# fluidex/plonkit

Hardware: AMD Instinct MI355X
Metric: G1 MSM throughput at 2^20 terms per GPU (KZG commitment of the PLONK prover) (higher is better)
Workload: dtype u256 (BN254 Fr/Fq Montgomery; 9x29-bit limbs in registers, v_mad_u64_u32); 1 GPU; Pippenger G1 MSM (KZG commitment), 2^20 uniform scalars per GPU, tau=42 monomial SRS sharded by rank (BASELINE configs[1]); terms_per_gpu=1048576, parallelism=srs-shard x1 + all_gather of partial sums, exchange=none (one GPU), pipeline_depth=3, settle_steps=0, comm_ranks=1

## Files before the change

plonkit_amd/csrc/ec29_dev.h:

```cpp
#pragma once
#include "field29_dev.h"
#include "ec_dev.h"

namespace plk {

struct AffW { FqW9 x, y; };
struct alignas(16) XyzzW { FqW9 x, y, zz, zzz; };

#define WM(a, b) mulw<FqW>((a), (b))
#define WS(a) sqrw<FqW>((a))
#define WMA(a, b, c, d) mul2addw<FqW>((a), (b), (c), (d))
#define LM(a, b) mulw_os<FqW>((a), (b))
#define LS(a) sqrw_os<FqW>((a))
#define LMA(a, b, c, d) mul2addw_os<FqW>((a), (b), (c), (d))

PLK_HD bool is_inf(const XyzzW &p) { return w_all_zero(p.zz); }
PLK_HD bool is_inf(const AffW &p) { return w_all_zero(p.x) && w_all_zero(p.y); }
PLK_HD XyzzW xyzzw_identity() { XyzzW r; r.x = w_zero<FqW>(); r.y = w_zero<FqW>(); r.zz = w_zero<FqW>(); r.zzz = w_zero<FqW>(); return r; }

PLK_HD XyzzW xyzzw_double_affine(const FqW9 &x, const FqW9 &y) {
    FqW9 u = addn(y, y), v = WS(u), w = WM(u, v), s = WM(x, v);
    FqW9 xx = WS(x), m = normw(addw(addw(xx, xx), xx));
    XyzzW r;
    r.x = sub4(WS(m), addn(s, s));
// ... 71 lines not shown
        }
        mulw2_add<FqW>(q.x, acc.zz, ax, yq, acc.zzz, ay, p, r);
    }
    if (maybe_zero_mod_p(p)) {
        AffW t; t.x = q.x; t.y = normw(yq);
        xyzzw_add_mixed_special(acc, t, false, p, r);
        fresh = is_inf(acc);
        return;
    }
    FqW9 pp, rr, ppp, qq;
    sqrw2<FqW>(p, r, pp, rr);
    mulw2<FqW>(p, pp, acc.x, pp, ppp, qq);
    FqW9 x3;
    {
#pragma unroll
        for (int i = 0; i < 9; i++) x3.l[i] = rr.l[i] + FqW::PAD4[i] - ppp.l[i] - 2 * qq.l[i];
        x3 = normw(x3);
    }
    FqW9 zz3, zzz3;
    mulw2<FqW>(acc.zz, pp, acc.zzz, ppp, zz3, zzz3);
    FqW9 t, nppp;
#pragma unroll
    for (int i = 0; i < 9; i++) { t.l[i] = qq.l[i] + FqW::PAD6N[i] - x3.l[i]; nppp.l[i] = FqW::PAD2N[i] - ppp.l[i]; }
    acc.y = WMA(r, t, acc.y, nppp);
    acc.x = x3;
    acc.zz = zz3;
    acc.zzz = zzz3;
}

PLK_HD void xyzzw_add(XyzzW &a, const XyzzW &b) {
    if (is_inf(b)) return;
    if (is_inf(a)) { a = b; return; }
    FqW9 u1 = LM(a.x, b.zz), u2 = LM(b.x, a.zz), s1 = LM(a.y, b.zzz), s2 = LM(b.y, a.zzz);
    FqW9 p = sub2(u2, u1), r = sub2(s2, s1);
    if (is_zero_mod_p(p)) {
        if (is_zero_mod_p(r)) a = xyzzw_double(a);
        else a = xyzzw_identity();
        return;
    }
    FqW9 pp = LS(p), ppp = LM(p, pp), qq = LM(u1, pp);
    FqW9 x3;
    {
        FqW9 rr = LS(r);
#pragma unroll
        for (int i = 0; i < 9; i++) x3.l[i] = rr.l[i] + FqW::PAD4[i] - ppp.l[i] - 2 * qq.l[i];
        x3 = normw(x3);
    }
    a.y = LMA(r, sub6(qq, x3), s1, neg2(ppp));
    a.x = x3;
    a.zz = LM(LM(a.zz, b.zz), pp);
    a.zzz = LM(LM(a.zzz, b.zzz), ppp);
}

__device__ __forceinline__ AffW load_affw(const G1Affine *p) {
    AffW r; r.x = unpack<FqW>(load_fp(&p->x)); r.y = unpack<FqW>(load_fp(&p->y)); return r;
}
__device__ __forceinline__ FqW9 load_w(const uint32_t *p) {
    FqW9 r;
    const u32x4 *q = reinterpret_cast<const u32x4 *>(p);
    u32x4 a = q[0], b = q[1];
    r.l[0] = a.x; r.l[1] = a.y; r.l[2] = a.z; r.l[3] = a.w; r.l[4] = b.x; r.l[5] = b.y; r.l[6] = b.z; r.l[7] = b.w; r.l[8] = p[8];
    return r;
}
__device__ __forceinline__ void store_w(uint32_t *p, const FqW9 &v) {
    u32x4 *q = reinterpret_cast<u32x4 *>(p);
    q[0] = u32x4{v.l[0], v.l[1], v.l[2], v.l[3]};
    q[1] = u32x4{v.l[4], v.l[5], v.l[6], v.l[7]};
    p[8] = v.l[8];
}
__device__ __forceinline__ XyzzW load_xyzzw(const XyzzW *p) {
    const uint32_t *w = reinterpret_cast<const uint32_t *>(p);
    XyzzW r;
    FqW9 *c[4] = {&r.x, &r.y, &r.zz, &r.zzz};
    u32x4 tail = *reinterpret_cast<const u32x4 *>(w + 32);
    const uint32_t t[4] = {tail.x, tail.y, tail.z, tail.w};
#pragma unroll
    for (int k = 0; k < 4; k++) {
        const u32x4 *q = reinterpret_cast<const u32x4 *>(w + 8 * k);
        u32x4 a = q[0], b = q[1];
        c[k]->l[0] = a.x; c[k]->l[1] = a.y; c[k]->l[2] = a.z; c[k]->l[3] = a.w;
        c[k]->l[4] = b.x; c[k]->l[5] = b.y; c[k]->l[6] = b.z; c[k]->l[7] = b.w; c[k]->l[8] = t[k];
    }
    return r;
}
__device__ __forceinline__ void store_xyzzw(XyzzW *p, const XyzzW &v) {
    uint32_t *w = reinterpret_cast<uint32_t *>(p);
    const FqW9 *c[4] = {&v.x, &v.y, &v.zz, &v.zzz};
#pragma unroll
    for (int k = 0; k < 4; k++) {
        u32x4 *q = reinterpret_cast<u32x4 *>(w + 8 * k);
        q[0] = u32x4{c[k]->l[0], c[k]->l[1], c[k]->l[2], c[k]->l[3]};
        q[1] = u32x4{c[k]->l[4], c[k]->l[5], c[k]->l[6], c[k]->l[7]};
    }
    *reinterpret_cast<u32x4 *>(w + 32) = u32x4{v.x.l[8], v.y.l[8], v.zz.l[8], v.zzz.l[8]};
}

__device__ __forceinline__ G1Xyzz xyzzw_export(const XyzzW &p) {
    G1Xyzz r;
    if (is_inf(p)) return xyzz_identity();
    r.x = pack<FqParams>(s_from_w(p.x)); r.y = pack<FqParams>(s_from_w(p.y));
    r.zz = pack<FqParams>(s_from_w(p.zz)); r.zzz = pack<FqParams>(s_from_w(p.zzz));
    return r;
}

}
```

plonkit_amd/csrc/field29_dev.h:

```cpp
#pragma once
#include "field_dev.h"
#include <utility>

namespace plk {

template <int... J, class F> __device__ __forceinline__ void static_for_impl(std::integer_sequence<int, J...>, F &&f) { (f(std::integral_constant<int, J>{}), ...); }
template <int N, class F> __device__ __forceinline__ void static_for(F &&f) { static_for_impl(std::make_integer_sequence<int, N>{}, static_cast<F &&>(f)); }

constexpr uint32_t M29 = (1u << 29) - 1;
constexpr uint32_t MULW_A_LIMB_MAX = 3280000000u;

struct FrW {
    static constexpr uint32_t P29[9] = {0x10000001u, 0x1f0fac9fu, 0x0e5c2450u, 0x07d090f3u, 0x1585d283u, 0x02db40c0u, 0x00a6e141u, 0x0e5c2634u, 0x0030644eu};
    static constexpr uint32_t INV29 = 0x0fffffffu;
    static constexpr uint32_t PINV0 = 0x10000001u;
    static constexpr uint32_t ONE_W[9] = {0x0fffff57u, 0x1ea70ab4u, 0x052c068bu, 0x17504f49u, 0x0aa8075bu, 0x1d4240ceu, 0x11d54c07u, 0x052ac7a8u, 0x000dc836u};
    static constexpr uint32_t W_FROM_S[9] = {0x0fffead7u, 0x1d5444f4u, 0x04438aa5u, 0x03b4d096u, 0x134c84dau, 0x0e92d304u, 0x14cb95b3u, 0x041b9d3du, 0x00058003u};
    static constexpr uint32_t S_FROM_W[9] = {0x0ffffffbu, 0x04b1a0e2u, 0x18334a6bu, 0x18ed2b3eu, 0x1462e36fu, 0x11b7bc3cu, 0x1cbd99bau, 0x183340fbu, 0x000e0a77u};
    static constexpr uint32_t PAD2[9] = {0x80000002u, 0x9e1f593bu, 0x9cb8489du, 0x8fa121e2u, 0x8b0ba502u, 0x85b6817du, 0x814dc27eu, 0x9cb84c64u, 0x0060c898u};
    static constexpr uint32_t PAD4[9] = {0x80000004u, 0x9c3eb27au, 0x9970913fu, 0x9f4243c9u, 0x96174a08u, 0x8b6d02feu, 0x829b8500u, 0x997098ccu, 0x00c19135u};
    static constexpr uint32_t PAD6[9] = {0x80000006u, 0x9a5e0bb9u, 0x9628d9e1u, 0x8ee365b0u, 0x8122ef0fu, 0x91238480u, 0x83e94782u, 0x9628e534u, 0x012259d2u};
    static constexpr uint32_t PAD8[9] = {0x80000008u, 0x987d64f8u, 0x92e12283u, 0x9e848797u, 0x8c2e9415u, 0x96da0601u, 0x85370a04u, 0x92e1319cu, 0x0183226fu};
};

// ... 416 lines not shown
    const uint32_t q = a.l[8] / (WP::P29[8] + 1u);
    W9<WP> r;
    int64_t c = 0;
#pragma unroll
    for (int i = 0; i < 8; i++) {
        const int64_t s = (int64_t)a.l[i] - (int64_t)q * (int64_t)WP::P29[i] + c;
        r.l[i] = (uint32_t)s & M29;
        c = s >> 29;
    }
    r.l[8] = (uint32_t)((int64_t)a.l[8] - (int64_t)q * (int64_t)WP::P29[8] + c);
    return csub_p(r);
}

template <class WP>
PLK_HD bool is_zero_mod_p(const W9<WP> &a) {
    uint32_t k = (a.l[0] * WP::PINV0) & M29;
    if (k >= 16) return false;
    return w_all_zero(reduce_full(a));
}

template <class WP>
PLK_HD bool maybe_zero_mod_p(const W9<WP> &a) { return ((a.l[0] * WP::PINV0) & M29) < 16; }

template <class WP>
PLK_HD W9<WP> mulsum3w(const W9<WP> &a0, const W9<WP> &b0, const W9<WP> &a1, const W9<WP> &b1, const W9<WP> &a2, const W9<WP> &b2) {
    uint32_t m[9];
    W9<WP> r;
    uint64_t acc = 0;
#pragma unroll
    for (int k = 0; k < 9; k++) {
#pragma unroll
        for (int i = 0; i <= k; i++) {
            acc += (uint64_t)a0.l[k - i] * b0.l[i]; PLK_CHAIN(acc); acc += (uint64_t)a1.l[k - i] * b1.l[i]; PLK_CHAIN(acc);
            acc += (uint64_t)a2.l[k - i] * b2.l[i]; PLK_CHAIN(acc);
        }
        PLK_MONT_LOW(k)
    }
#pragma unroll
    for (int k = 9; k < 17; k++) {
#pragma unroll
        for (int i = k - 8; i <= 8; i++) {
            acc += (uint64_t)a0.l[k - i] * b0.l[i]; PLK_CHAIN(acc); acc += (uint64_t)a1.l[k - i] * b1.l[i]; PLK_CHAIN(acc);
            acc += (uint64_t)a2.l[k - i] * b2.l[i]; PLK_CHAIN(acc);
        }
        PLK_MONT_HIGH(k)
    }
    r.l[8] = (uint32_t)acc;
    return r;
}

template <class WP> PLK_HD W9<WP> w_from_s(const W9<WP> &raw) { return mulw(raw, w_from_s_const<WP>()); }
template <class WP> PLK_HD W9<WP> s_from_w(const W9<WP> &a) { return csub_p(mulw(a, s_from_w_const<WP>())); }

using FrW9 = W9<FrW>;
using FqW9 = W9<FqW>;

}
```

plonkit_amd/csrc/msm.hip:

```cpp
#include "msm_shape.h"
#include "msm.h"
#include "ec29_quad_dev.h"
#include "comm.h"
#include "hostmath.h"
#include <cstring>
#include <cstdlib>

namespace plk {

int32_t msm_small_launch(plk_ctx::MsmSlot &S, hipStream_t stream, const G1Affine *bases, uint32_t copy_stride, const ScalarSet &set,
                         uint32_t batch, uint32_t n, bool ev_on, void *host_out);
constexpr uint32_t SM_PLANES_HOST = 17;
constexpr uint64_t MSM_SMALL_MAX = 1ull << 15;
constexpr uint64_t MSM_OWNED_MAX = 1ull << 16;

__global__ void __launch_bounds__(MSM_THREADS) msm_digits(ScalarSet set, MsmParams p, int32_t *digits) {
    const uint32_t i = blockIdx.x * MSM_THREADS + threadIdx.x, m = blockIdx.y;
    if (i >= p.n) return;
    Fr k = to_canonical(load_fp(set.v[m] + i));
    uint32_t carry = 0;
    const uint32_t half = 1u << (p.c - 1);
    int32_t *out = digits + (size_t)m * p.windows * p.n + i;
    for (uint32_t w = 0; w < p.windows; w++) {
        uint32_t v = extract_bits(k.l, w * p.c, p.c) + carry;
// ... 68 lines not shown
        lcnt[b] = 0;
    }
    __syncthreads();
#pragma unroll
    for (uint32_t k = 0; k < PER; k++) {
        const int32_t d = dreg[k];
        if (d) {
            const uint32_t i = first + tid + k * PART_THREADS;
            uint32_t mg = (uint32_t)(d < 0 ? -d : d) - 1, bin = mg >> p.fine_bits;
            staged[lstart[bin] + atomicAdd(&lcnt[bin], 1u)] = ((copy_tag | i) << 8) | (d < 0 ? 0x80u : 0u) | (mg & ((1u << p.fine_bits) - 1));
        }
    }
    __syncthreads();
    copy_out_runs<PART_THREADS>(lstart, gbase, staged, entries, p.nbins);
}

__global__ void __launch_bounds__(1024) msm_scan_bins(uint32_t *hist, uint32_t *bin_start, uint32_t *task_start, uint32_t total_bins) {
    __shared__ uint32_t sums[1024], tsums[1024];
    const uint32_t tid = threadIdx.x;
    const uint32_t per = (total_bins + 1023) / 1024;
    uint32_t lo = tid * per, hi = lo + per < total_bins ? lo + per : total_bins, s = 0, ts = 0;
    if (lo > total_bins) lo = total_bins;
    for (uint32_t i = lo; i < hi; i++) { s += hist[i]; ts += (hist[i] + TASK_MAX - 1) / TASK_MAX; }
    sums[tid] = s; tsums[tid] = ts;
    __syncthreads();
    for (uint32_t off = 1; off < 1024; off <<= 1) {
        uint32_t v = tid >= off ? sums[tid - off] : 0, tv = tid >= off ? tsums[tid - off] : 0;
        __syncthreads();
        sums[tid] += v; tsums[tid] += tv;
        __syncthreads();
    }
    uint32_t run = tid ? sums[tid - 1] : 0, trun = tid ? tsums[tid - 1] : 0;
    for (uint32_t i = lo; i < hi; i++) {
        uint32_t c = hist[i];
        bin_start[i] = run; run += c;
        task_start[i] = trun; trun += (c + TASK_MAX - 1) / TASK_MAX;
        hist[i] = 0;
    }
    if (tid == 1023) { bin_start[total_bins] = sums[1023]; task_start[total_bins] = tsums[1023]; }
}

constexpr int RC_THREADS = 1024, RC_SCALARS = 1024;
static_assert(RC_WINDOWS == 254 / 17 + 1, "the fused path is the c = 17 shape");

__device__ __forceinline__ bool wave_same_scalar(const Fr &k, bool live, uint64_t live_mask) {
    const int leader = __ffsll((unsigned long long)live_mask) - 1;
    uint32_t diff = 0;
#pragma unroll
    for (int i = 0; i < 8; i++) diff |= k.l[i] ^ (uint32_t)__shfl((int)k.l[i], leader);
    return __ballot(live && diff != 0) == 0;
}

constexpr int RC_COUNT_PER = 4;
__global__ void __launch_bounds__(RC_THREADS) msm_recode_count(ScalarSet set, MsmParams p, uint32_t *hist) {
    __shared__ uint32_t lcnt[1024];
    const uint32_t tid = threadIdx.x, m = blockIdx.y;
    lcnt[tid] = 0;
    __syncthreads();
    Fr k[RC_COUNT_PER];
    bool live[RC_COUNT_PER];
#pragma unroll
    for (int r = 0; r < RC_COUNT_PER; r++) {
        const uint32_t i = (blockIdx.x * RC_COUNT_PER + r) * RC_THREADS + tid;
        live[r] = i < p.n;
        if (live[r]) k[r] = load_fp(set.v[m] + i);
    }
#pragma unroll
    for (int r = 0; r < RC_COUNT_PER; r++) {
        const uint64_t lv = __ballot(live[r]);
        if (!lv) continue;
        const bool same = wave_same_scalar(k[r], live[r], lv);
        if (!live[r]) continue;
        int32_t d[RC_WINDOWS];
        recode17(to_canonical(k[r]), d);
        if (same) {
            if ((tid & 63) == (uint32_t)(__ffsll((unsigned long long)lv) - 1)) {
#pragma unroll
                for (uint32_t w = 0; w < RC_WINDOWS; w++)
                    if (d[w]) { const uint32_t mg = (uint32_t)(d[w] < 0 ? -d[w] : d[w]) - 1; atomicAdd(&lcnt[mg >> p.fine_bits], (uint32_t)__popcll(lv)); }
            }
            continue;
        }
#pragma unroll
        for (uint32_t w = 0; w < RC_WINDOWS; w++)
            if (d[w]) { const uint32_t mg = (uint32_t)(d[w] < 0 ? -d[w] : d[w]) - 1; atomicAdd(&lcnt[mg >> p.fine_bits], 1u); }
    }
    __syncthreads();
    if (tid < p.nbins && lcnt[tid]) atomicAdd(&hist[m * p.nbins + tid], lcnt[tid]);
}

__global__ void __launch_bounds__(RC_THREADS) msm_recode_scatter(ScalarSet set, MsmParams p, uint32_t *cursor, const uint32_t *bin_start, uint32_t *entries) {
    extern __shared__ __attribute__((aligned(16))) char smem[];
    uint32_t *lcnt = reinterpret_cast<uint32_t *>(smem);
    uint32_t *lstart = lcnt + p.nbins;
    uint32_t *gbase = lstart + p.nbins + 1;
    uint32_t *staged = gbase + p.nbins;
    const uint32_t tid = threadIdx.x, m = blockIdx.y;
    const uint32_t i = blockIdx.x * RC_SCALARS + tid;
    cursor += m * p.nbins; bin_start += m * p.nbins;
    int32_t d[RC_WINDOWS];
    const bool live = i < p.n;
    const uint64_t lv = __ballot(live);
    bool same = false;
    uint32_t lane_rank = 0, wave_live = 0;
    if (live) {
        const Fr k = load_fp(set.v[m] + i);
        same = wave_same_scalar(k, true, lv);
        recode17(to_canonical(k), d);
        lane_rank = (uint32_t)__popcll(lv & ((1ull << (tid & 63)) - 1)); wave_live = (uint32_t)__popcll(lv);
    } else {
#pragma unroll
        for (uint32_t w = 0; w < RC_WINDOWS; w++) d[w] = 0;
    }
    for (uint32_t b = tid; b < p.nbins; b += RC_THREADS) lcnt[b] = 0;
    __syncthreads();
    uint32_t at[RC_WINDOWS];
#pragma unroll
    for (uint32_t w = 0; w < RC_WINDOWS; w++) {
        at[w] = 0;
        if (d[w]) {
            const uint32_t mg = (uint32_t)(d[w] < 0 ? -d[w] : d[w]) - 1;
            if (!same) at[w] = atomicAdd(&lcnt[mg >> p.fine_bits], 1u);
            else {
                uint32_t base = 0;
                if (lane_rank == 0) base = atomicAdd(&lcnt[mg >> p.fine_bits], wave_live);
                at[w] = (uint32_t)__shfl((int)base, __ffsll((unsigned long long)lv) - 1) + lane_rank;
            }
        }
    }
    __syncthreads();
    {
        const uint32_t cnt = tid < p.nbins ? lcnt[tid] : 0;
        uint32_t v = cnt;
        for (int off = 1; off < 64; off <<= 1) { uint32_t t = __shfl_up(v, off); if ((int)(tid & 63) >= off) v += t; }
        uint32_t *wtot = gbase;
        if ((tid & 63) == 63) wtot[tid >> 6] = v;
        __syncthreads();
        uint32_t before = 0;
        for (uint32_t w = 0; w < (tid >> 6); w++) before += wtot[w];
        __syncthreads();
        const uint32_t reserved = cnt ? bin_start[tid] + atomicAdd(&cursor[tid], cnt) : 0;
        if (tid < p.nbins) lstart[tid] = before + v - cnt;
        if (tid == RC_THREADS - 1) lstart[p.nbins] = before + v;
        __syncthreads();
        if (tid < p.nbins) gbase[tid] = reserved;
    }
    const uint32_t fmask = (1u << p.fine_bits) - 1;
#pragma unroll
    for (uint32_t w = 0; w < RC_WINDOWS; w++) {
        if (!d[w]) continue;
        const uint32_t mg = (uint32_t)(d[w] < 0 ? -d[w] : d[w]) - 1, bin = mg >> p.fine_bits;
        staged[lstart[bin] + at[w]] = ((((uint32_t)w << p.nbits) | i) << 8) | (d[w] < 0 ? 0x80u : 0u) | (mg & fmask);
    }
    __syncthreads();
    copy_out_runs<RC_THREADS>(lstart, gbase, staged, entries, p.nbins);
}

__device__ __forceinline__ XyzzW shfl_xor_w(const XyzzW &v, int mask) {
    XyzzW r;
#pragma unroll
    for (int i = 0; i < 9; i++) {
// ... 129 lines not shown
        PLK_HIP(hipMemsetAsync(found.p, 0, sizeof(uint32_t), stream));
        hipLaunchKernelGGL(table_find_inf_kernel, dim3(fblocks), dim3(256), 0, stream, (const G1Affine *)table, total, found.as<uint32_t>());
        hipError_t e = hipMemcpyAsync(&found_host, found.p, sizeof(uint32_t), hipMemcpyDeviceToHost, stream);
        if (e == hipSuccess) e = hipStreamSynchronize(stream);
        found.release();
        PLK_HIP(e);
    }
    PLK_HIP(hipGetLastError());
    ctx->srs_w_valid = true;
    ctx->srs_w_copies = copies;
    ctx->srs_w_no_inf = found_host == 0;
    return PLK_OK;
}

static uint32_t slots_per_task(uint32_t fb) { return (1u << fb) + 2 * MSM_THREADS; }
static uint32_t meta_per_task(uint32_t fb) { return (1u << fb) + 2; }

constexpr uint32_t HOT_SPAN = 8;
__device__ __forceinline__ uint32_t bucket_span(const uint32_t *meta, uint32_t b, uint32_t mu) {
    const uint32_t s0 = meta[b], e0 = meta[b + 1];
    return e0 > s0 ? (e0 - 1) / mu - s0 / mu : 0;
}
__device__ __forceinline__ void latency_chain_priority() { __builtin_amdgcn_s_setprio(3); }

template <uint32_t FB, uint32_t RL_LOG>
__global__ void __launch_bounds__(MSM_THREADS) msm_fold_hot(XyzzW *partials, const uint32_t *task_meta, const uint32_t *task_start, uint32_t total_bins) {
    constexpr uint32_t FINE = Shape<FB>::FINE, SLOT_PRIMARY = Shape<FB>::SLOT_PRIMARY, SLOT_HEAD = Shape<FB>::SLOT_HEAD,
                       SLOTS_PER_TASK = Shape<FB>::SLOTS_PER_TASK, META_PER_TASK = Shape<FB>::META_PER_TASK, RL = 1u << RL_LOG, RB = FINE / RL;
    latency_chain_priority();
    const uint32_t gt = blockIdx.x * MSM_THREADS + threadIdx.x;
    const uint32_t task = gt / RL, sub = gt % RL;
    const bool live = task < task_start[total_bins];
    const uint32_t *meta = task_meta + (size_t)(live ? task : 0) * META_PER_TASK;
    const uint32_t nc_raw = live ? meta[FINE + 1] : 0, nc = nc_raw & ~TASK_OWNED_BIT;
    if (!__any(nc != 0 && !(nc_raw & TASK_OWNED_BIT))) return;
    const uint32_t mu = (nc_raw & TASK_OWNED_BIT) ? 0x7fffffffu : (nc ? (nc + MSM_THREADS - 1) / MSM_THREADS : 1);
    uint32_t hot_mask = 0;
    if (nc) for (uint32_t k = 0; k < RB; k++) if (bucket_span(meta, RB * sub + k, mu) > HOT_SPAN) hot_mask |= 1u << k;
    if (!__any(hot_mask != 0)) return;
    XyzzW *P = partials + (size_t)(live ? task : 0) * SLOTS_PER_TASK;
    for (uint32_t owner = 0; owner < RL; owner++) {
        const uint32_t m = __shfl(hot_mask, owner, RL);
        for (uint32_t k = 0; k < RB; k++) {
            if (!((m >> k) & 1)) continue;
            const uint32_t b = RB * owner + k, tf = meta[b] / mu, tl = (meta[b + 1] - 1) / mu;
            XyzzW acc = xyzzw_identity();
            for (uint32_t t = tf + 1 + sub; t <= tl; t += RL) { XyzzW o = load_xyzzw(P + SLOT_HEAD + t); xyzzw_add_nl(acc, o); }
            for (uint32_t x = 1; x < RL; x <<= 1) { XyzzW o = shfl_xor_w(acc, x); xyzzw_add_nl(acc, o); }
            if (sub == 0) store_xyzzw(P + SLOT_PRIMARY + b, acc);
        }
    }
}

template <uint32_t FB, uint32_t RL_LOG>
__global__ void __launch_bounds__(MSM_THREADS, 2) msm_task_reduce(const XyzzW *partials, const uint32_t *task_meta,
                                                                   const uint32_t *task_start, XyzzW *task_out, uint32_t total_bins) {
    constexpr uint32_t FINE = Shape<FB>::FINE, SLOT_PRIMARY = Shape<FB>::SLOT_PRIMARY, SLOT_HEAD = Shape<FB>::SLOT_HEAD, SLOT_TAIL = Shape<FB>::SLOT_TAIL,
                       SLOTS_PER_TASK = Shape<FB>::SLOTS_PER_TASK, META_PER_TASK = Shape<FB>::META_PER_TASK, RL = 1u << RL_LOG, RB = FINE / RL, RB_LOG = FB - RL_LOG;
    static_assert(FB >= RL_LOG + 1, "at least two buckets per lane");
    latency_chain_priority();
    const uint32_t gt = blockIdx.x * MSM_THREADS + threadIdx.x;
    const uint32_t task = gt / RL, sub = gt % RL;
    const bool live = task < task_start[total_bins];
    if (!__any(live)) return;
    const uint32_t *meta = task_meta + (size_t)(live ? task : 0) * META_PER_TASK;
    const uint32_t nc_raw = live ? meta[FINE + 1] : 0, nc = nc_raw & ~TASK_OWNED_BIT;
    const uint32_t mu = (nc_raw & TASK_OWNED_BIT) ? 0x7fffffffu : (nc ? (nc + MSM_THREADS - 1) / MSM_THREADS : 1);
    const XyzzW *P = partials + (size_t)(live ? task : 0) * SLOTS_PER_TASK;
    XyzzW X = xyzzw_identity(), Y = xyzzw_identity();
    uint32_t k = nc ? RB : 0;
    uint32_t piece = 0, piece_end = 0;
    bool pending_sum = false;
    constexpr uint32_t USTEPS = RL_LOG + RB_LOG + 1 + RL_LOG;
    uint32_t ustep = 0;
    for (;;) {
        const bool done = (piece >= piece_end) && !pending_sum && k == 0;
        const bool lockstep = __all(done);
        if (lockstep && ustep == USTEPS) break;
        XyzzW O = xyzzw_identity();
        bool to_y = false;
        if (!lockstep) {
            if (piece < piece_end) { O = load_xyzzw(P + piece); piece++; }
            else if (pending_sum) { to_y = true; pending_sum = false; }
            else if (k > 0) {
                k--;
                const uint32_t b = RB * sub + k, s0 = meta[b], e0 = meta[b + 1];
                if (e0 > s0) {
                    const uint32_t tf = s0 / mu, tl = (e0 - 1) / mu;
                    pending_sum = true;
                    if (tf == tl) O = load_xyzzw(P + SLOT_PRIMARY + b);
                    else {
                        O = load_xyzzw(P + SLOT_TAIL + tf);
                        if (tl - tf > HOT_SPAN) { piece = SLOT_PRIMARY + b; piece_end = piece + 1; }
                        else { piece = SLOT_HEAD + tf + 1; piece_end = SLOT_HEAD + tl + 1; }
                    }
                } else to_y = true;
            }
        } else {
            if (ustep < RL_LOG) {
                const uint32_t off = 1u << ustep;
                O = shfl_down_w(X, off);
                if (sub + off >= RL) O = xyzzw_identity();
            } else {
                if (ustep == RL_LOG) {
                    if (live && sub == 0) store_xyzzw(task_out + 2 * (size_t)task + 1, X);
                    if (sub == 0) X = xyzzw_identity();
                }
                if (ustep < RL_LOG + RB_LOG) O = X;
                else if (ustep == RL_LOG + RB_LOG) O = Y;
                else O = shfl_xor_w(X, 1 << (ustep - RL_LOG - RB_LOG - 1));
            }
            ustep++;
        }
        if (to_y) O = Y;
        XyzzW Tacc = X;
        xyzzw_add(Tacc, O);
        if (to_y) Y = Tacc; else X = Tacc;
    }
    if (live && sub == 0) store_xyzzw(task_out + 2 * (size_t)task, X);
}

template <uint32_t FB>
__global__ void __launch_bounds__(MSM_THREADS) msm_task_reduce_quad(const XyzzW *partials, const uint32_t *task_meta, const uint32_t *task_start, XyzzW *task_out, uint32_t total_bins) {
    constexpr uint32_t FINE = Shape<FB>::FINE, SLOT_PRIMARY = Shape<FB>::SLOT_PRIMARY, SLOT_HEAD = Shape<FB>::SLOT_HEAD, SLOT_TAIL = Shape<FB>::SLOT_TAIL,
                       SLOTS_PER_TASK = Shape<FB>::SLOTS_PER_TASK, META_PER_TASK = Shape<FB>::META_PER_TASK, RL_LOG = 4, RL = 1u << RL_LOG, RB = FINE / RL, RB_LOG = FB - RL_LOG;
    latency_chain_priority();
    const uint32_t task = blockIdx.x * (MSM_THREADS / 64) + (threadIdx.x >> 6), sub = (threadIdx.x & 63u) >> 2, coord = threadIdx.x & 3u;
    const bool live = task < task_start[total_bins];
    if (!live) return;
    const uint32_t *meta = task_meta + (size_t)(live ? task : 0) * META_PER_TASK;
    const uint32_t nc_raw = live ? meta[FINE + 1] : 0, nc = nc_raw & ~TASK_OWNED_BIT;
    const uint32_t mu = (nc_raw & TASK_OWNED_BIT) ? 0x7fffffffu : (nc ? (nc + MSM_THREADS - 1) / MSM_THREADS : 1);
    const XyzzW *P = partials + (size_t)(live ? task : 0) * SLOTS_PER_TASK;
    FqW9 X = w_zero<FqW>(), Y = w_zero<FqW>();
    uint32_t k = nc ? RB : 0;
    uint32_t piece = 0, piece_end = 0;
    bool pending_sum = false;
    constexpr uint32_t USTEPS = RL_LOG + RB_LOG + 1 + RL_LOG;
    uint32_t ustep = 0;
    for (;;) {
        const bool done = (piece >= piece_end) && !pending_sum && k == 0;
        const bool lockstep = __all(done);
        if (lockstep && ustep == USTEPS) break;
        FqW9 O = w_zero<FqW>();
        bool to_y = false;
        if (!lockstep) {
            if (piece < piece_end) { O = load_coord(P + piece, coord); piece++; }
            else if (pending_sum) { to_y = true; pending_sum = false; }
            else if (k > 0) {
                k--;
                const uint32_t b = RB * sub + k, s0 = meta[b], e0 = meta[b + 1];
                if (e0 > s0) {
                    const uint32_t tf = s0 / mu, tl = (e0 - 1) / mu;
                    pending_sum = true;
                    if (tf == tl) O = load_coord(P + SLOT_PRIMARY + b, coord);
                    else {
                        O = load_coord(P + SLOT_TAIL + tf, coord);
                        if (tl - tf > HOT_SPAN) { piece = SLOT_PRIMARY + b; piece_end = piece + 1; }
                        else { piece = SLOT_HEAD + tf + 1; piece_end = SLOT_HEAD + tl + 1; }
                    }
                } else to_y = true;
            }
        } else {
            if (ustep < RL_LOG) {
                const uint32_t off = 1u << ustep;
#pragma unroll
                for (int i = 0; i < 9; i++) O.l[i] = __shfl_down(X.l[i], 4 * off);
                if (sub + off >= RL) O = w_zero<FqW>();
            } else {
// ... 122 lines not shown
    if (S.pinned) (void)hipHostFree(S.pinned);
    S.pinned = nullptr; S.pinned_cap = 0;
    PLK_HIP(hipHostMalloc(&S.pinned, bytes, hipHostMallocDefault));
    S.pinned_cap = bytes;
    return PLK_OK;
}

struct BigArgs { const G1Affine *bases; uint64_t srs_n; uint32_t copies, c_bits, nbits; ScalarSet set; uint32_t batch; uint64_t n; bool no_inf = false; };
static int32_t msm_big_launch(plk_ctx *ctx, plk_ctx::MsmSlot &S, hipStream_t stream, const BigArgs &A) {
    const G1Affine *bases = A.bases;
    const uint32_t batch = A.batch, copies = A.copies;
    const uint64_t n = A.n;
    MsmParams p;
    p.n = (uint32_t)n;
    p.c = A.c_bits;
    p.windows = 254 / p.c + 1;
    p.groups = p.windows / copies;
    p.nbits = A.nbits;
    p.copy_stride = copies > 1 ? (uint32_t)(p.groups * A.srs_n) : 0;
    p.fine_bits = FINE_BITS;
    p.coarse_bits = p.c - 1 - p.fine_bits;
    p.nbins = 1u << p.coarse_bits;
    p.batch = batch;
    const ScalarSet &set = A.set;
    const uint32_t total_sets = batch * p.groups, total_bins = total_sets * p.nbins, total_windows = batch * p.windows;
    const uint32_t max_tasks = total_bins + (uint32_t)(((uint64_t)total_windows * n) / TASK_MAX) + 1;
    PLK_TRY(S.a.reserve((size_t)(3 * total_bins + 4) * sizeof(uint32_t)));
    PLK_TRY(S.b.reserve((size_t)total_windows * n * sizeof(uint32_t)));
    const uint32_t META_PER_TASK = meta_per_task(p.fine_bits), SLOTS_PER_TASK = slots_per_task(p.fine_bits);
    PLK_TRY(S.c.reserve((size_t)max_tasks * 2 * sizeof(XyzzW) + (size_t)max_tasks * META_PER_TASK * 4));
    PLK_TRY(S.e.reserve((size_t)max_tasks * SLOTS_PER_TASK * sizeof(XyzzW)));
    PLK_TRY(S.d.reserve((size_t)13 * total_sets * sizeof(G1Xyzz)));
    uint32_t *hist = S.a.as<uint32_t>(), *bin_start = hist + total_bins, *task_start = bin_start + total_bins + 1;
    uint32_t *entries = S.b.as<uint32_t>();
    XyzzW *task_out = S.c.as<XyzzW>();
    uint32_t *task_meta = reinterpret_cast<uint32_t *>(task_out + 2 * (size_t)max_tasks);
    XyzzW *partials = S.e.as<XyzzW>();
    G1Xyzz *window_out = S.d.as<G1Xyzz>();

    PLK_HIP(hipMemsetAsync(hist, 0, total_bins * sizeof(uint32_t), stream));
    static std::atomic<bool> attr_set{false};
    if (!attr_set) {
        PLK_HIP(hipFuncSetAttribute(reinterpret_cast<const void *>(msm_partition<true>), hipFuncAttributeMaxDynamicSharedMemorySize, 96 * 1024));
        PLK_HIP(hipFuncSetAttribute(reinterpret_cast<const void *>(msm_recode_scatter), hipFuncAttributeMaxDynamicSharedMemorySize, 96 * 1024));
        PLK_TRY(msm_accumulate_prepare());
        attr_set = true;
    }
    static const bool fused_ok = [] { const char *e = getenv("PLK_MSM_FUSED_RECODE"); return !(e && e[0] == '0'); }();
    const uint32_t shape_prephase = (fused_ok && p.groups == 1 && p.c == 17 && p.windows == RC_WINDOWS && p.nbins <= 1024) ? 1u : 2u;
    if (shape_prephase == 1) {
        const uint32_t cblocks = (uint32_t)((n + (uint64_t)RC_THREADS * RC_COUNT_PER - 1) / ((uint64_t)RC_THREADS * RC_COUNT_PER));
        const uint32_t sblocks = (uint32_t)((n + RC_SCALARS - 1) / RC_SCALARS);
        const size_t lds = (size_t)(3 * p.nbins + 1 + RC_SCALARS * RC_WINDOWS) * sizeof(uint32_t);
        hipLaunchKernelGGL(msm_recode_count, dim3(cblocks, batch), dim3(RC_THREADS), 0, stream, set, p, hist);
        hipLaunchKernelGGL(msm_scan_bins, dim3(1), dim3(1024), 0, stream, hist, bin_start, task_start, total_bins);
        hipLaunchKernelGGL(msm_recode_scatter, dim3(sblocks, batch), dim3(RC_THREADS), lds, stream, set, p, hist, (const uint32_t *)bin_start, entries);
    } else {
        PLK_TRY(S.f.reserve((size_t)total_windows * n * sizeof(int32_t)));
        int32_t *digits = S.f.as<int32_t>();
        hipLaunchKernelGGL(msm_digits, dim3((uint32_t)((n + MSM_THREADS - 1) / MSM_THREADS), batch), dim3(MSM_THREADS), 0, stream, set, p, digits);
        const uint32_t pblocks = (uint32_t)((n + DIGIT_CHUNK - 1) / DIGIT_CHUNK);
        const size_t plds_count = (size_t)p.nbins * sizeof(uint32_t);
        const size_t plds_scatter = (size_t)(3 * p.nbins + 1 + DIGIT_CHUNK) * sizeof(uint32_t);
        hipLaunchKernelGGL(msm_partition<false>, dim3(pblocks, total_windows), dim3(PART_THREADS), plds_count, stream, (const int32_t *)digits, p, hist, (const uint32_t *)nullptr, (uint32_t *)nullptr);
        hipLaunchKernelGGL(msm_scan_bins, dim3(1), dim3(1024), 0, stream, hist, bin_start, task_start, total_bins);
        hipLaunchKernelGGL(msm_partition<true>, dim3(pblocks, total_windows), dim3(PART_THREADS), plds_scatter, stream, (const int32_t *)digits, p, hist, (const uint32_t *)bin_start, entries);
    }
    if (ctx->ev_on) PLK_HIP(hipEventRecord(S.ev[0], stream));
    const uint32_t shape_variant = n <= MSM_OWNED_MAX ? 2u : 0u;
    S.acc_no_inf = shape_variant == 0 && A.no_inf;
    msm_accumulate_launch((int)shape_variant, S.acc_no_inf, max_tasks, stream, bases, (const uint32_t *)entries, (const uint32_t *)bin_start, (const uint32_t *)task_start, partials, task_meta, p);
    if (ctx->ev_on) (void)hipEventRecord(S.ev[1], stream);
    (void)hipEventRecord(S.acc_done, stream);
    const bool others_in_flight = ctx->msm_enq != ctx->msm_fin;
    const uint32_t shape_lanes = (total_sets == 1 && !others_in_flight) ? 4u : ((batch >= 3 || others_in_flight) ? 16u : 32u);
    const uint32_t rblocks = (max_tasks * (shape_lanes == 16 ? 16u : 32u) + MSM_THREADS - 1) / MSM_THREADS;
    constexpr uint32_t FB = FINE_BITS;
    if (shape_lanes == 4) {
        hipLaunchKernelGGL((msm_fold_hot<FB, 5>), dim3(rblocks), dim3(MSM_THREADS), 0, stream, partials, (const uint32_t *)task_meta, (const uint32_t *)task_start, total_bins);
        hipLaunchKernelGGL((msm_task_reduce_quad<FB>), dim3((max_tasks + MSM_THREADS / 64 - 1) / (MSM_THREADS / 64)), dim3(MSM_THREADS), 0, stream,
                           (const XyzzW *)partials, (const uint32_t *)task_meta, (const uint32_t *)task_start, task_out, total_bins);
    } else if (shape_lanes == 16) {
        hipLaunchKernelGGL((msm_fold_hot<FB, 4>), dim3(rblocks), dim3(MSM_THREADS), 0, stream, partials, (const uint32_t *)task_meta, (const uint32_t *)task_start, total_bins);
        hipLaunchKernelGGL((msm_task_reduce<FB, 4>), dim3(rblocks), dim3(MSM_THREADS), 0, stream,
                           (const XyzzW *)partials, (const uint32_t *)task_meta, (const uint32_t *)task_start, task_out, total_bins);
    } else {
        hipLaunchKernelGGL((msm_fold_hot<FB, 5>), dim3(rblocks), dim3(MSM_THREADS), 0, stream, partials, (const uint32_t *)task_meta, (const uint32_t *)task_start, total_bins);
        hipLaunchKernelGGL((msm_task_reduce<FB, 5>), dim3(rblocks), dim3(MSM_THREADS), 0, stream,
                           (const XyzzW *)partials, (const uint32_t *)task_meta, (const uint32_t *)task_start, task_out, total_bins);
    }
    hipLaunchKernelGGL(msm_bin_fold, dim3((total_bins + MSM_THREADS / 64 - 1) / (MSM_THREADS / 64)), dim3(MSM_THREADS), 0, stream, task_out, (const uint32_t *)task_start, total_bins);
    const uint32_t roles = WS_FIRST_F_ROLE + (p.nbins + MSM_THREADS - 1) / MSM_THREADS - 1 + 1;
    hipLaunchKernelGGL(msm_window_sums_quad, dim3(total_sets, roles), dim3(MSM_THREADS), 0, stream, (const XyzzW *)task_out, (const uint32_t *)task_start, window_out, p.nbins, roles);
    PLK_HIP(hipGetLastError());
    PLK_TRY(slot_pinned(S, (size_t)roles * total_sets * sizeof(G1Xyzz)));
    PLK_HIP(hipMemcpyAsync(S.pinned, window_out, (size_t)roles * total_sets * sizeof(G1Xyzz), hipMemcpyDeviceToHost, stream));
    S.roles = roles;
    S.windows = p.groups;
    S.c_bits = p.c;
    S.fine_bits = p.fine_bits;
    plk_msm_shape &sh = S.shape;
    sh.table_copies = copies; sh.window_bits = p.c; sh.windows = p.windows; sh.bucket_sets = p.groups;
    sh.fine_bits = p.fine_bits; sh.coarse_bins = p.nbins;
    sh.accumulate_variant = shape_variant; sh.prephase = shape_prephase; sh.reduce_lanes = shape_lanes;
    return PLK_OK;
}

static int32_t msm_naive_launch(plk_ctx::MsmSlot &S, hipStream_t stream, const BigArgs &A) {
    const uint32_t blocks = (uint32_t)((A.n + MSM_THREADS - 1) / MSM_THREADS);
    PLK_TRY(S.d.reserve((size_t)A.batch * blocks * sizeof(G1Xyzz)));
    for (uint32_t m = 0; m < A.batch; m++)
        hipLaunchKernelGGL(msm_naive, dim3(blocks), dim3(MSM_THREADS), 0, stream, A.bases, A.set.v[m], (uint32_t)A.n, S.d.as<G1Xyzz>() + (size_t)m * blocks);
    PLK_HIP(hipGetLastError());
    (void)hipEventRecord(S.acc_done, stream);
    S.pending_parts = blocks;
    S.windows = 0;
    S.c_bits = 0;
    PLK_TRY(slot_pinned(S, (size_t)A.batch * blocks * sizeof(G1Xyzz)));
    PLK_HIP(hipMemcpyAsync(S.pinned, S.d.p, (size_t)A.batch * blocks * sizeof(G1Xyzz), hipMemcpyDeviceToHost, stream));
    return PLK_OK;
}

int32_t msm_enqueue_batch(plk_ctx *ctx, const Fr *const *scalars_dev, uint32_t batch, uint64_t n, uint64_t base_offset, hipStream_t caller) {
    if (ctx->msm_enq - ctx->msm_fin >= plk_ctx::MSM_SLOTS) { set_error("msm: " + std::to_string(plk_ctx::MSM_SLOTS) + " commitments are already in flight (call the finish function first)"); return PLK_ERR_ARG; }
    uint32_t slot_index = 0;
    while (ctx->slot[slot_index].busy) slot_index++;
    plk_ctx::MsmSlot &S = ctx->slot[slot_index];
    auto in_flight = [&]() { ctx->fifo[ctx->msm_enq % plk_ctx::MSM_SLOTS] = (uint8_t)slot_index; S.busy = true; ctx->msm_enq++; };
    if (!S.stream) {
        int lo_prio = 0, hi_prio = 0;
        PLK_HIP(hipDeviceGetStreamPriorityRange(&lo_prio, &hi_prio));
        PLK_HIP(hipStreamCreateWithPriority(&S.stream, hipStreamNonBlocking, hi_prio));
        PLK_HIP(hipEventCreateWithFlags(&S.ready, hipEventDisableTiming));
        PLK_HIP(hipEventCreateWithFlags(&S.acc_done, hipEventDisableTiming));
    }
    if (ctx->ev_on && !S.ev[0]) { PLK_HIP(hipEventCreate(&S.ev[0])); PLK_HIP(hipEventCreate(&S.ev[1])); }
    PLK_HIP(hipEventRecord(S.ready, caller));
// ... 331 lines not shown
```

plonkit_amd/csrc/msm_shape.h:

```cpp
#pragma once
#include "ctx.h"
#include "ec_dev.h"
#include "ec29_dev.h"

namespace plk {

constexpr int MSM_THREADS = 256;
constexpr uint32_t FINE_BITS = 6;
constexpr uint32_t CHUNK = 16384;
constexpr uint32_t DIGIT_CHUNK = 16384;
constexpr uint32_t TASK_MAX = CHUNK;

constexpr uint32_t MSM_MAX_BATCH = 8;

struct MsmParams {
    uint32_t n;
    uint32_t c;
    uint32_t windows;
    uint32_t fine_bits;
    uint32_t coarse_bits;
    uint32_t nbins;
    uint32_t batch;
    uint32_t groups;
    uint32_t nbits;
    uint32_t copy_stride;
};

struct ScalarSet { const Fr *v[MSM_MAX_BATCH]; };

PLK_HD uint32_t extract_bits(const uint32_t *k, uint32_t pos, uint32_t c) {
    uint32_t limb = pos >> 5, off = pos & 31;
    if (limb >= 8) return 0;
    uint64_t v = k[limb];
    if (limb + 1 < 8) v |= (uint64_t)k[limb + 1] << 32;
    return (uint32_t)(v >> off) & ((1u << c) - 1);
}
constexpr int RC_WINDOWS = 15;
PLK_HD void recode17(const Fr &k, int32_t (&d)[RC_WINDOWS]) {
    uint32_t carry = 0;
#pragma unroll
    for (uint32_t w = 0; w < RC_WINDOWS; w++) {
        const uint32_t v = extract_bits(k.l, w * 17, 17) + carry;
        if (v >= (1u << 16) && w + 1 < RC_WINDOWS) { d[w] = (int32_t)v - (1 << 17); carry = 1; } else { d[w] = (int32_t)v; carry = 0; }
    }
}

template <uint32_t FB> struct Shape {
    static constexpr uint32_t FINE = 1u << FB;
    static constexpr uint32_t SLOT_PRIMARY = 0, SLOT_HEAD = FINE, SLOT_TAIL = FINE + MSM_THREADS, SLOTS_PER_TASK = FINE + 2 * MSM_THREADS;
    static constexpr uint32_t META_PER_TASK = FINE + 2;
};

constexpr uint32_t TASK_OWNED_BIT = 0x80000000u;

int32_t msm_accumulate_prepare();
void msm_accumulate_launch(int variant, bool no_inf, uint32_t max_tasks, hipStream_t stream, const G1Affine *bases, const uint32_t *entries,
                           const uint32_t *bin_start, const uint32_t *task_start, XyzzW *partials, uint32_t *task_meta, const MsmParams &p);

}
```

Baseline: 888.9 Mscalar·mul/s.

## Cache canonical scalars across recode passes and pair multiplies in task reduce

The recode-count kernel now converts each scalar from Montgomery form to canonical form once, using a 29-bit-limb reduction. It writes the result to a scratch buffer, so the scatter kernel reads canonical scalars and skips a second conversion. A new XYZZ add variant pairs independent field multiplies (mulw2/mulw2_add) to expose more instruction-level parallelism, and it is enabled for the 16-lane task-reduce path. The cost is extra global memory traffic of one scalar store and load per term, plus scratch space of batch*n field elements.

```diff
diff --git a/plonkit_amd/csrc/ec29_dev.h b/plonkit_amd/csrc/ec29_dev.h
--- a/plonkit_amd/csrc/ec29_dev.h
+++ b/plonkit_amd/csrc/ec29_dev.h
@@ -147,6 +147,43 @@
     a.zzz = LM(LM(a.zzz, b.zzz), ppp);
 }
 
+PLK_HD void xyzzw_add_pairs(XyzzW &a, const XyzzW &b) {
+    if (is_inf(b)) return;
+    if (is_inf(a)) { a = b; return; }
+    FqW9 u1, s1, p, r;
+    mulw2<FqW>(a.x, b.zz, a.y, b.zzz, u1, s1);
+    {
+        FqW9 nu, ns;
+#pragma unroll
+        for (int i = 0; i < 9; i++) { nu.l[i] = FqW::PAD2[i] - u1.l[i]; ns.l[i] = FqW::PAD2[i] - s1.l[i]; }
+        mulw2_add<FqW>(b.x, a.zz, nu, b.y, a.zzz, ns, p, r);
+    }
+    if (is_zero_mod_p(p)) {
+        if (is_zero_mod_p(r)) a = xyzzw_double(a);
+        else a = xyzzw_identity();
+        return;
+    }
+    FqW9 zz12, zzz12;
+    mulw2<FqW>(a.zz, b.zz, a.zzz, b.zzz, zz12, zzz12);
+    FqW9 pp, rr, ppp, qq;
+#pragma unroll
+    for (int i = 0; i < 9; i++) { PLK_CHAIN(p.l[i]); PLK_CHAIN(r.l[i]); }
+    sqrw2<FqW>(p, r, pp, rr);
+    mulw2<FqW>(p, pp, u1, pp, ppp, qq);
+    FqW9 x3;
+    {
+#pragma unroll
+        for (int i = 0; i < 9; i++) x3.l[i] = rr.l[i] + FqW::PAD4[i] - ppp.l[i] - 2 * qq.l[i];
+        x3 = normw(x3);
+    }
+    FqW9 t, nppp;
+#pragma unroll
+    for (int i = 0; i < 9; i++) { t.l[i] = qq.l[i] + FqW::PAD6N[i] - x3.l[i]; nppp.l[i] = FqW::PAD2N[i] - ppp.l[i]; }
+    a.y = WMA(r, t, s1, nppp);
+    a.x = x3;
+    mulw2<FqW>(zz12, pp, zzz12, ppp, a.zz, a.zzz);
+}
+
 __device__ __forceinline__ AffW load_affw(const G1Affine *p) {
     AffW r; r.x = unpack<FqW>(load_fp(&p->x)); r.y = unpack<FqW>(load_fp(&p->y)); return r;
 }
diff --git a/plonkit_amd/csrc/field29_dev.h b/plonkit_amd/csrc/field29_dev.h
--- a/plonkit_amd/csrc/field29_dev.h
+++ b/plonkit_amd/csrc/field29_dev.h
@@ -492,6 +492,24 @@
 template <class WP> PLK_HD W9<WP> w_from_s(const W9<WP> &raw) { return mulw(raw, w_from_s_const<WP>()); }
 template <class WP> PLK_HD W9<WP> s_from_w(const W9<WP> &a) { return csub_p(mulw(a, s_from_w_const<WP>())); }
 
+template <class WP, class PR>
+PLK_HD W9<WP> canonical_w(const Fp<PR> &s) {
+    const W9<WP> a = unpack<WP>(s);
+    uint32_t m[9];
+    W9<WP> r;
+    uint64_t acc = 0;
+#pragma unroll
+    for (int k = 0; k < 9; k++) {
+        acc += (uint64_t)a.l[k] << 5;
+        PLK_MONT_LOW(k)
+    }
+#pragma unroll
+    for (int k = 9; k < 17; k++) PLK_MONT_HIGH(k)
+    r.l[8] = (uint32_t)acc;
+    return csub_p(r);
+}
+PLK_HD W9<FrW> fr_canonical_w(const Fr &k) { return canonical_w<FrW>(k); }
+
 using FrW9 = W9<FrW>;
 using FqW9 = W9<FqW>;
 
diff --git a/plonkit_amd/csrc/msm.hip b/plonkit_amd/csrc/msm.hip
--- a/plonkit_amd/csrc/msm.hip
+++ b/plonkit_amd/csrc/msm.hip
@@ -144,7 +144,7 @@
 }
 
 constexpr int RC_COUNT_PER = 4;
-__global__ void __launch_bounds__(RC_THREADS) msm_recode_count(ScalarSet set, MsmParams p, uint32_t *hist) {
+__global__ void __launch_bounds__(RC_THREADS) msm_recode_count(ScalarSet set, MsmParams p, uint32_t *hist, Fr *canon) {
     __shared__ uint32_t lcnt[1024];
     const uint32_t tid = threadIdx.x, m = blockIdx.y;
     lcnt[tid] = 0;
@@ -164,7 +164,11 @@
         const bool same = wave_same_scalar(k[r], live[r], lv);
         if (!live[r]) continue;
         int32_t d[RC_WINDOWS];
-        recode17(to_canonical(k[r]), d);
+        {
+            const FrW9 kc = fr_canonical_w(k[r]);
+            store_fp(canon + (size_t)m * p.n + (blockIdx.x * RC_COUNT_PER + r) * RC_THREADS + tid, pack<FrParams>(kc));
+            recode17_w(kc, d);
+        }
         if (same) {
             if ((tid & 63) == (uint32_t)(__ffsll((unsigned long long)lv) - 1)) {
 #pragma unroll
@@ -181,7 +185,7 @@
     if (tid < p.nbins && lcnt[tid]) atomicAdd(&hist[m * p.nbins + tid], lcnt[tid]);
 }
 
-__global__ void __launch_bounds__(RC_THREADS) msm_recode_scatter(ScalarSet set, MsmParams p, uint32_t *cursor, const uint32_t *bin_start, uint32_t *entries) {
+__global__ void __launch_bounds__(RC_THREADS) msm_recode_scatter(const Fr *canon, MsmParams p, uint32_t *cursor, const uint32_t *bin_start, uint32_t *entries) {
     extern __shared__ __attribute__((aligned(16))) char smem[];
     uint32_t *lcnt = reinterpret_cast<uint32_t *>(smem);
     uint32_t *lstart = lcnt + p.nbins;
@@ -196,9 +200,9 @@
     bool same = false;
     uint32_t lane_rank = 0, wave_live = 0;
     if (live) {
-        const Fr k = load_fp(set.v[m] + i);
+        const Fr k = load_fp(canon + (size_t)m * p.n + i);
         same = wave_same_scalar(k, true, lv);
-        recode17(to_canonical(k), d);
+        recode17(k, d);
         lane_rank = (uint32_t)__popcll(lv & ((1ull << (tid & 63)) - 1)); wave_live = (uint32_t)__popcll(lv);
     } else {
 #pragma unroll
@@ -434,7 +438,7 @@
     }
 }
 
-template <uint32_t FB, uint32_t RL_LOG>
+template <uint32_t FB, uint32_t RL_LOG, bool PAIRS = false>
 __global__ void __launch_bounds__(MSM_THREADS, 2) msm_task_reduce(const XyzzW *partials, const uint32_t *task_meta,
                                                                    const uint32_t *task_start, XyzzW *task_out, uint32_t total_bins) {
     constexpr uint32_t FINE = Shape<FB>::FINE, SLOT_PRIMARY = Shape<FB>::SLOT_PRIMARY, SLOT_HEAD = Shape<FB>::SLOT_HEAD, SLOT_TAIL = Shape<FB>::SLOT_TAIL,
@@ -496,7 +500,7 @@
         }
         if (to_y) O = Y;
         XyzzW Tacc = X;
-        xyzzw_add(Tacc, O);
+        if constexpr (PAIRS) xyzzw_add_pairs(Tacc, O); else xyzzw_add(Tacc, O);
         if (to_y) Y = Tacc; else X = Tacc;
     }
     if (live && sub == 0) store_xyzzw(task_out + 2 * (size_t)task, X);
@@ -725,9 +729,11 @@
         const uint32_t cblocks = (uint32_t)((n + (uint64_t)RC_THREADS * RC_COUNT_PER - 1) / ((uint64_t)RC_THREADS * RC_COUNT_PER));
         const uint32_t sblocks = (uint32_t)((n + RC_SCALARS - 1) / RC_SCALARS);
         const size_t lds = (size_t)(3 * p.nbins + 1 + RC_SCALARS * RC_WINDOWS) * sizeof(uint32_t);
-        hipLaunchKernelGGL(msm_recode_count, dim3(cblocks, batch), dim3(RC_THREADS), 0, stream, set, p, hist);
+        PLK_TRY(S.f.reserve((size_t)batch * n * sizeof(Fr)));
+        Fr *canon = S.f.as<Fr>();
+        hipLaunchKernelGGL(msm_recode_count, dim3(cblocks, batch), dim3(RC_THREADS), 0, stream, set, p, hist, canon);
         hipLaunchKernelGGL(msm_scan_bins, dim3(1), dim3(1024), 0, stream, hist, bin_start, task_start, total_bins);
-        hipLaunchKernelGGL(msm_recode_scatter, dim3(sblocks, batch), dim3(RC_THREADS), lds, stream, set, p, hist, (const uint32_t *)bin_start, entries);
+        hipLaunchKernelGGL(msm_recode_scatter, dim3(sblocks, batch), dim3(RC_THREADS), lds, stream, (const Fr *)canon, p, hist, (const uint32_t *)bin_start, entries);
     } else {
         PLK_TRY(S.f.reserve((size_t)total_windows * n * sizeof(int32_t)));
         int32_t *digits = S.f.as<int32_t>();
@@ -755,7 +761,7 @@
                            (const XyzzW *)partials, (const uint32_t *)task_meta, (const uint32_t *)task_start, task_out, total_bins);
     } else if (shape_lanes == 16) {
         hipLaunchKernelGGL((msm_fold_hot<FB, 4>), dim3(rblocks), dim3(MSM_THREADS), 0, stream, partials, (const uint32_t *)task_meta, (const uint32_t *)task_start, total_bins);
-        hipLaunchKernelGGL((msm_task_reduce<FB, 4>), dim3(rblocks), dim3(MSM_THREADS), 0, stream,
+        hipLaunchKernelGGL((msm_task_reduce<FB, 4, true>), dim3(rblocks), dim3(MSM_THREADS), 0, stream,
                            (const XyzzW *)partials, (const uint32_t *)task_meta, (const uint32_t *)task_start, task_out, total_bins);
     } else {
         hipLaunchKernelGGL((msm_fold_hot<FB, 5>), dim3(rblocks), dim3(MSM_THREADS), 0, stream, partials, (const uint32_t *)task_meta, (const uint32_t *)task_start, total_bins);
diff --git a/plonkit_amd/csrc/msm_shape.h b/plonkit_amd/csrc/msm_shape.h
--- a/plonkit_amd/csrc/msm_shape.h
+++ b/plonkit_amd/csrc/msm_shape.h
@@ -44,6 +44,17 @@
         if (v >= (1u << 16) && w + 1 < RC_WINDOWS) { d[w] = (int32_t)v - (1 << 17); carry = 1; } else { d[w] = (int32_t)v; carry = 0; }
     }
 }
+PLK_HD void recode17_w(const FrW9 &k, int32_t (&d)[RC_WINDOWS]) {
+    uint32_t carry = 0;
+#pragma unroll
+    for (uint32_t w = 0; w < RC_WINDOWS; w++) {
+        const uint32_t limb = (w * 17) / 29, off = (w * 17) % 29;
+        uint32_t v = k.l[limb] >> off;
+        if (off + 17 > 29 && limb + 1 < 9) v |= k.l[limb + 1] << (29 - off);
+        v = (v & ((1u << 17) - 1)) + carry;
+        if (v >= (1u << 16) && w + 1 < RC_WINDOWS) { d[w] = (int32_t)v - (1 << 17); carry = 1; } else { d[w] = (int32_t)v; carry = 0; }
+    }
+}
 
 template <uint32_t FB> struct Shape {
     static constexpr uint32_t FINE = 1u << FB;
```

Result: faster. 906.3 Mscalar·mul/s (median of 6 runs) (+2.0%).
